# churchill-lab/alntools

Hardware: AMD Instinct MI355X
Metric: alignments/sec BAM->EC (100M PE reads, 8-hap) at 1/2/4/8 MI355X (higher is better)
Workload: dtype u32

## Files before the change

### alntools_amd/csrc/ecb.hip

```cpp
#include <hip/hip_runtime.h>

#include <algorithm>
#include <climits>
#include <cstddef>
#include <cstdarg>
#include <cstdio>
#include <cstring>
#include <cstdlib>
#include <memory>
#include <mutex>
#include <string>
#include <vector>

#include "../../include/ecb.h"

namespace {

typedef unsigned long long u64;
typedef unsigned int u32;
typedef unsigned short u16;

constexpr int TPB = 256;
constexpr u32 MAX_PROBE = 256;
constexpr u32 PENDING = 0xFFFFFFFFu;
constexpr u32 ARENA_CHUNK = 512;
constexpr u32 QSTRIPES = 64;
constexpr u32 ARENA_REGIONS = 64;
constexpr u32 MAX_LOCI = (1u << 26) - 2u;
constexpr u32 MAX_LOCI_SHORT = (1u << 25) - 2u;
constexpr u32 INL = 5;
constexpr u32 DEAD_KEY = 0xFFFFFFFFu;
constexpr u32 SPIN_MAX = 1u << 16;

constexpr u32 ERR_CONTRACT = 1u;
constexpr u32 ERR_RANGE = 2u;
constexpr u32 ERR_ARENA = 4u;
constexpr u32 ERR_QUEUE = 8u;
constexpr u32 ERR_INTERNAL = 16u;
constexpr u32 ERR_COUNT = 32u;

struct alignas(64) Slot {
    u64 lo;
    u32 n1;
    u32 off;
    u32 count;
    u32 first_inv;
    uint2 pair[INL];
};
static_assert(sizeof(Slot) == 64, "one EC per 64-byte line");
static_assert(offsetof(Slot, n1) == 8 && offsetof(Slot, off) == 12 && offsetof(Slot, count) == 16 && offsetof(Slot, first_inv) == 20,
              "k_count_bins reads {n1, off} and {count, first_inv} as 8-byte words");
struct Entry {
    u64 lo, reserved;
    u32 count, first_inv;
    u32 off, n;
};
static_assert(sizeof(Entry) == 32, "exchange format");

struct Counters {
    u64 all, valid;
    u64 arena_top;
    u64 n_queue;
    u64 n_queue_s[QSTRIPES];
    u64 n_ecs;
    u32 err;
    u32 full;
    u64 arena_reg[ARENA_REGIONS];
    u64 next_slice;
    u64 n_mismatch;
    u32 last_rid, pad_;
    u64 n_probe_tiles;
};

__host__ __device__ __forceinline__ u32 arena_regions(u64 arena_cap) { return (u32)(arena_cap >> 16 >= ARENA_REGIONS ? ARENA_REGIONS : (arena_cap >> 16 ? arena_cap >> 16 : 1)); }
__device__ __forceinline__ u64 arena_alloc(Counters* ctr, u64 arena_cap, u32 n, u32 hint) {
    const u32 R = arena_regions(arena_cap);
    const u64 per = arena_cap / R;
    for (u32 t = 0; t < R; ++t) {
        const u32 r = (hint + t) % R;
        const u64 at = atomicAdd(&ctr->arena_reg[r], (u64)n);
        if (at + n <= (u64)(r + 1) * per) return at;
    }
    return ~0ull;
}

__device__ __forceinline__ u32 fmix32(u32 h) {
    h ^= h >> 16; h *= 0x85EBCA6Bu;
    h ^= h >> 13; h *= 0xC2B2AE35u;
    h ^= h >> 16;
    return h;
}
__device__ __forceinline__ u64 pair_hash64(u32 locus, u32 mask) {
    const u32 h0 = fmix32(locus * 0x9E3779B1u + mask * 0x85EBCA77u + 0x7F4A7C15u);
    const u32 h1 = fmix32((h0 ^ locus) * 0xC2B2AE3Du + mask);
    return ((u64)h1 << 32) | h0;
}
__device__ __forceinline__ u64 finish_hash(u64 s0, u32 n) { return (s0 + ((u64)n << 32) + n) | 1ull; }

__device__ __forceinline__ bool rec_valid(u32 hf) {
    if (hf & 0x4u) return false;
    if (hf & 0x1u) {
        if ((hf & 0x80u) || !(hf & 0x2u) || (hf & (ECB_FLAG_MATE_OTHER_REF | ECB_FLAG_NEXT_POS_NEG))) return false;
    }
    return true;
}

enum { ST_NONE = 0, ST_LOOK, ST_HIT, ST_CREATED, ST_PENDING, ST_FULL, ST_OTHER, ST_STUCK };
enum { CMP_EQUAL = 0, CMP_DIFFERENT, CMP_INCOMPLETE, CMP_UNSURE };
struct SlotView { u32 n, off; uint2 p[INL]; };

__device__ __forceinline__ u64 fresh64(u64* p) { return atomicOr(p, 0ull); }
__device__ __forceinline__ void store_wt64(u64* p, u64 v) { __hip_atomic_store(p, v, __ATOMIC_RELAXED, __HIP_MEMORY_SCOPE_AGENT); }
__device__ __forceinline__ u64 pack2(uint2 v) { return ((u64)v.y << 32) | v.x; }
__device__ __forceinline__ uint2 unpack2(u64 v) { return make_uint2((u32)v, (u32)(v >> 32)); }
__device__ __forceinline__ void publish_key(Slot* s, u32 n1, u32 off) { store_wt64(reinterpret_cast<u64*>(&s->n1), ((u64)off << 32) | n1); }
__device__ __forceinline__ uint2 key_pair(const Slot& s, const uint2* arena, u32 i) { return i < INL ? s.pair[i] : arena[(u64)s.off + (i - INL)]; }
__device__ __forceinline__ uint2 key_pair_fresh(Slot* s, uint2* arena, u32 off, u32 i) {
    return unpack2(fresh64(reinterpret_cast<u64*>(i < INL ? &s->pair[i] : arena + ((u64)off + (i - INL)))));
}

__device__ __forceinline__ SlotView make_view(uint4 a, uint4 b, uint4 c, uint4 d) {
    SlotView v;
    v.n = a.z - 1u; v.off = a.w;
    v.p[0] = make_uint2(b.z, b.w); v.p[1] = make_uint2(c.x, c.y); v.p[2] = make_uint2(c.z, c.w);
    v.p[3] = make_uint2(d.x, d.y); v.p[4] = make_uint2(d.z, d.w);
    return v;
}
constexpr u32 RANKED_MAX = 16;
template <class F>
__device__ __forceinline__ void ranked_pairs(const SlotView& v, const uint2* arena, F&& emit) {
    const u32 sn = v.n;
    u32 X[RANKED_MAX], Y[RANKED_MAX];
#pragma unroll
    for (u32 i = 0; i < INL; ++i) { X[i] = i < sn ? v.p[i].x : 0xFFFFFFFFu; Y[i] = v.p[i].y; }
    if (sn <= INL) {
#pragma unroll
        for (u32 i = 0; i < INL; ++i) {
            u32 r = 0;
#pragma unroll
            for (u32 j = 0; j < INL; ++j) r += X[j] < X[i] ? 1u : 0u;
            if (i < sn) emit(r, X[i], Y[i]);
        }
    } else {
#pragma unroll
        for (u32 k = 0; k < RANKED_MAX - INL; ++k) {
            const uint2 t = INL + k < sn ? arena[(u64)v.off + k] : make_uint2(0xFFFFFFFFu, 0u);
            X[INL + k] = t.x; Y[INL + k] = t.y;
        }
#pragma unroll
        for (u32 i = 0; i < RANKED_MAX; ++i) {
            u32 r = 0;
#pragma unroll
            for (u32 j = 0; j < RANKED_MAX; ++j) r += X[j] < X[i] ? 1u : 0u;
            if (i < sn) emit(r, X[i], Y[i]);
        }
    }
}
constexpr u32 BIG_LDS = 2048;
template <class F>
__device__ __forceinline__ void ranked_pairs_wave(const Slot& s, const uint2* arena, u32 sn, u32* sx, u32 lane, F&& emit) {
    const bool in_lds = sn <= BIG_LDS;
    if (in_lds) {
        for (u32 i = lane; i < sn; i += 64) sx[i] = key_pair(s, arena, i).x;
        __builtin_amdgcn_fence(__ATOMIC_ACQ_REL, "wavefront");
        __builtin_amdgcn_wave_barrier();
    }
    for (u32 i = lane; i < sn; i += 64) {
        const uint2 pi = key_pair(s, arena, i);
        u32 r = 0;
        if (in_lds) {
            u32 j = 0;
            for (; j + 4u <= sn; j += 4u) {
                const uint4 v = *reinterpret_cast<const uint4*>(&sx[j]);
                r += (v.x < pi.x ? 1u : 0u) + (v.y < pi.x ? 1u : 0u) + (v.z < pi.x ? 1u : 0u) + (v.w < pi.x ? 1u : 0u);
            }
            for (; j < sn; ++j) r += sx[j] < pi.x ? 1u : 0u;
        } else {
            for (u32 j = 0; j < sn; ++j) r += key_pair(s, arena, j).x < pi.x;
        }
        emit(r, pi.x, pi.y);
    }
    if (in_lds) {
        __builtin_amdgcn_fence(__ATOMIC_ACQ_REL, "wavefront");
        __builtin_amdgcn_wave_barrier();
    }
}
template <class Cmp>
__device__ __forceinline__ int table_lookup(Slot* table, u64 cap_mask, u64 lo, u64& j, u32& probes, const Cmp& cmp, u32 abl = 0u, u32* first_inv_seen = nullptr) {
    for (; probes < MAX_PROBE; ++probes, j = (j + 1) & cap_mask) {
        Slot* s = table + j;
// ... 2253 lines not shown
    HIPCHK(h, hipMemsetAsync(&h->ctr->full, 0, sizeof(u32), h->stream));
    HIPCHK(h, hipMemsetAsync(&h->ctr->next_slice, 0, sizeof(u64), h->stream));
    return ECB_OK;
}

int launch_stream(ecb_handle* h, StreamVariant v, const StreamPlan& P, const u32* d_rid, const u32* d_loc, const u32* d_hf, const int* d_pos, u64 n,
                  u32 prev_rid, const u32* d_last, u32 launch, u64 offered, u64* timing = nullptr) {
    const bool verify = v == SV_VERIFY;
    int2* const rng = verify ? nullptr : (int2*)h->rng;
    u64* d_resume = nullptr; u32* d_wcounts = nullptr;
    POOL(h, P_RESUME, d_resume, 2 * P.slices);
    if (!launch) k_init_resume<<<nblk(P.slices, TPB), TPB, 0, h->stream>>>(d_resume, P.slices, P.chunk, verify ? nullptr : (Counters*)h->ctr);
    POOL(h, P_WCOUNTS, d_wcounts, 3 * P.pwaves);
    if (launch) RCCHK(zero_launch_words(h));
    else {
        if (verify) {
            HIPCHK(h, hipMemsetAsync(d_wcounts, 0, 3 * P.pwaves * sizeof(u32), h->stream));
            RCCHK(zero_launch_words(h));
            HIPCHK(h, hipMemsetAsync(&h->ctr->n_mismatch, 0, sizeof(u64), h->stream));
        } else if (h->wave_arena_n < P.pwaves) {
            HIPCHK(h, h->wave_arena.grow(2 * P.pwaves * sizeof(u64), 0, 2 * h->wave_arena_n * sizeof(u64), h->stream));
            h->wave_arena_n = P.pwaves;
        }
        *h->pin_cold = StreamCold{h->arena, h->arena_cap, h->queue, h->queue_cap, d_resume, d_wcounts, verify ? nullptr : (u64*)h->wave_arena, timing,
                                  P.chunk, prev_rid, d_pos, rng, verify ? 0u : h->cfg.n_loci, verify ? 0u : h->cfg.n_haplotypes};
        HIPCHK(h, hipMemcpyAsync(h->d_cold, h->pin_cold.get(), sizeof(StreamCold), hipMemcpyHostToDevice, h->stream));
    }
    const StreamArgs a{d_rid, d_loc, d_hf, n, h->table, h->cap - 1, h->ctr, h->read_slot, h->run.reads_hi, h->d_cold,
                       !verify && getenv("ECB_ABLATE") ? (u32)atoi(getenv("ECB_ABLATE")) : 0u, d_pos, rng};
    if (h->prof && !verify) hipEventRecord(h->ev0, h->stream);
    STREAM_VARIANTS[v].kernel<<<(unsigned)P.blocks, TPB, 0, h->stream>>>(a);
    if (h->prof && !verify) hipEventRecord(h->ev1, h->stream);
    k_sum_counts<<<1, 1024, 0, h->stream>>>(d_wcounts, P.pwaves, h->ctr, verify ? 1u : 0u, offered, h->queue_cap, d_last);
    HIPCHK(h, hipGetLastError());
    if (!verify) h->last_variant = v;
    return ECB_OK;
}

int verify_pass(ecb_handle* h, const StreamPlan& P, const u32* d_rid, const u32* d_loc, const u32* d_hf, u64 n, u32 prev_rid, u64* n_long, u32 tw) {
    RCCHK(launch_stream(h, SV_VERIFY, P, d_rid, d_loc, d_hf, nullptr, n, prev_rid, nullptr, 0, 0));
    RCCHK(sync_counters(h));
    return run_deferred(h, d_rid, d_loc, d_hf, n, true, tw, n_long);
}
int verify_batch(ecb_handle* h, const u32* d_rid, const u32* d_loc, const u32* d_hf, u64 n, u32 prev_rid, u64* n_mismatch, u64* n_long, u32 tw = 512u) {
    StreamPlan P;
    RCCHK(plan_stream(h, n, &P, SV_VERIFY));
    u64 nq = 0;
    if (const int rc = verify_pass(h, P, d_rid, d_loc, d_hf, n, prev_rid, &nq, tw); rc != ECB_OK) {
        if (h->hctr.err) {
            const std::string refusal = h->err;
            HIPCHK(h, hipMemsetAsync(&h->ctr->err, 0, sizeof(u32), h->stream));
            HIPCHK(h, hipMemsetAsync(&h->ctr->n_queue, 0, (1 + QSTRIPES) * sizeof(u64), h->stream));
            h->hctr.err = 0; h->hctr.n_queue = 0;
            h->err = refusal;
        }
        return rc;
    }
    *n_mismatch = h->hctr.n_mismatch;
    *n_long = nq;
    HIPCHK(h, hipMemsetAsync(&h->ctr->n_queue, 0, (1 + QSTRIPES) * sizeof(u64), h->stream));
    h->hctr.n_queue = 0;
    return ECB_OK;
}

int build_batch(ecb_handle* h, const u32* d_rid, const u32* d_loc, const u32* d_hf, const int* d_pos, u64 n, u32 tw, bool* launched) {
    if (n == 0) return ECB_OK;
    const bool hinted = h->reads_hint != 0;
    u32 last_rid = 0;
    u64 reads_after = std::max<u64>(h->reads_hint, h->run.n_reads);
    if (!hinted) {
        HIPCHK(h, hipMemcpyAsync(&last_rid, d_rid + rec_at(n - 1, tw), sizeof(u32), hipMemcpyDeviceToHost, h->stream));
        HIPCHK(h, hipStreamSynchronize(h->stream));
        reads_after = (u64)(u32)(last_rid + 1u);
        if (reads_after < h->run.n_reads) return fail(h, ECB_ERR_CONTRACT, "read_id went backwards across pushes");
    }
    RCCHK(ensure_read_slot(h, reads_after));
    h->run.reads_hi = reads_after;
    while (h->n_ecs() * 2 > h->cap) { RCCHK(grow_table(h, h->cap * 4)); }
    const StreamVariant v = pick_variant(h, n);
    StreamPlan P;
    RCCHK(plan_stream(h, n, &P, v));
    u64* timing = nullptr;
#ifdef ECB_TIMING
    HIPCHK(h, hipMalloc(&timing, 8 * sizeof(u64)));
    HIPCHK(h, hipMemset(timing, 0, 8 * sizeof(u64)));
#endif
    h->ctr_synced = false;
    *launched = true;
    const u64 probe_before = h->hctr.n_probe_tiles;
    int rc = ECB_OK;
    for (u32 launch = 0;; ++launch) {
        rc = launch_stream(h, v, P, d_rid, d_loc, d_hf, d_pos, n, h->run.prev_rid, d_rid + rec_at(n - 1, tw), launch, launch ? 0 : n, timing);
        if (rc != ECB_OK) break;
        rc = sync_counters(h);
        if (h->prof) {
            float ms = 0; hipEventElapsedTime(&ms, h->ev0, h->ev1);
            h->prof_ms += ms; h->prof_launches += 1;
        }
        if (rc != ECB_OK) break;
        const bool parked = h->hctr.full != 0;
        rc = run_deferred(h, d_rid, d_loc, d_hf, n, false, tw);
        if (rc != ECB_OK) break;
        if (!parked) break;
        rc = grow_table(h, h->cap * 4);
        if (rc != ECB_OK) break;
    }
#ifdef ECB_TIMING
    {
        u64 t[8];
        hipMemcpy(t, timing, sizeof(t), hipMemcpyDeviceToHost); hipFree(timing);
        static const char* nm[8] = {"(a) filter+heads", "tile decisions", "prefetch issue+clear+geometry", "(b) LDS tables", "hash entries", "(c) lookup", "publish/settle/slot stores", "-"};
        u64 tot = 0; for (int i = 0; i < 7; ++i) tot += t[i];
        fprintf(stderr, "[ecb timing] %llu waves, clocks per wave:", (unsigned long long)P.slices);
        for (int i = 0; i < 7; ++i) fprintf(stderr, "  %s %.0f (%.1f%%)", nm[i], (double)t[i] / P.slices, 100.0 * t[i] / std::max<u64>(tot, 1));
        fprintf(stderr, "  tile visits on the probe-on path %llu of %llu tiles", (unsigned long long)t[7], (unsigned long long)((n + WT - 1) / WT));
        fprintf(stderr, "\n");
    }
#endif
    RCCHK(rc);
    {
        const u64 tiles = (n + WT - 1) / WT, on_path = h->hctr.n_probe_tiles - probe_before;
        if (on_path * 4 > tiles) h->par_stream = true; else if (on_path * 16 < tiles) h->par_stream = false;
    }
    if (h->prof) h->prof_records += n;
    if (h->cfg.flags & ECB_F_VERIFY) {
        u64 bad = 0, nl = 0;
        RCCHK(verify_batch(h, d_rid, d_loc, d_hf, n, h->run.prev_rid, &bad, &nl, tw));
        h->run.n_mismatch += bad;
        if (bad) return fail(h, ECB_ERR_VERIFY, "exactness pass: %llu read(s) of this batch sit in an EC whose key is not their target set", (unsigned long long)bad);
    }
    if (hinted) {
        last_rid = h->hctr.last_rid;
        reads_after = (u64)(u32)(last_rid + 1u);
        if (reads_after < h->run.n_reads) return fail(h, ECB_ERR_CONTRACT, "read_id went backwards across pushes");
    }
    h->run.prev_rid = last_rid;
    h->run.n_reads = reads_after;
    h->run.records_pushed += n;
    return ECB_OK;
}
int process_batch(ecb_handle* h, const u32* d_rid, const u32* d_loc, const u32* d_hf, const int* d_pos, u64 n, u32 tw = 512u) {
    bool launched = false;
    const int rc = build_batch(h, d_rid, d_loc, d_hf, d_pos, n, tw, &launched);
    return launched ? run_refused(h, rc) : rc;
}

int ensure_staging(ecb_handle* h, u64 need) {
    if (need <= h->st_cap) return ECB_OK;
    h->st_loc = h->st_hf = nullptr; h->st_pos = nullptr; h->st_cap = 0;
    const u64 cap = std::max<u64>(need, h->cfg.max_batch_records);
    const u64 stride = (cap * sizeof(u32) + (2ull << 20) - 1) / (2ull << 20) * (2ull << 20) / sizeof(u32);
    const bool rg = (h->cfg.flags & ECB_F_RANGES) != 0;
    HIPCHK(h, h->st_rid.alloc((rg ? 4 : 3) * stride * sizeof(u32)));
    h->st_cap = cap;
    h->st_loc = h->st_rid + stride; h->st_hf = h->st_rid + 2 * stride;
    if (rg) h->st_pos = reinterpret_cast<int*>(h->st_rid + 3 * stride);
    return ECB_OK;
}

int stage_and_process(ecb_handle* h, const u32* rid, const u32* loc, const u32* hf, const int* pos, u64 m) {
    const u64 nc = h->run.c_rid.size();
    const u64 n = nc + m;
    if (!n) return ECB_OK;
    RCCHK(ensure_staging(h, n));
    const bool rg = (h->cfg.flags & ECB_F_RANGES) != 0;
    const struct { void* st; const void *carry, *window; } streams[4] = {
        {h->st_rid, h->run.c_rid.data(), rid}, {h->st_loc, h->run.c_loc.data(), loc}, {h->st_hf, h->run.c_hf.data(), hf}, {h->st_pos, h->run.c_pos.data(), pos}};
    for (int w = 0; w < 2; ++w)
        for (int i = 0; i < (rg ? 4 : 3) && (w ? m : nc); ++i)
            HIPCHK(h, hipMemcpyAsync((u32*)streams[i].st + (w ? nc : 0), w ? streams[i].window : streams[i].carry, (w ? m : nc) * 4, hipMemcpyHostToDevice, h->stream));
    HIPCHK(h, hipStreamSynchronize(h->stream));
    h->run.c_rid.clear(); h->run.c_loc.clear(); h->run.c_hf.clear(); h->run.c_pos.clear();
    return process_batch(h, h->st_rid, h->st_loc, h->st_hf, rg ? h->st_pos : nullptr, n);
}

int excl_scan_dev(ecb_handle* h, const u32* in, u64 n, u32* out, u64* d_total, u32 stride = 1, u32* last32 = nullptr) {
    u32* sums = nullptr;
    POOL(h, P_SUMS, sums, scan_words(n));
    HIPCHK(h, scan_launch(h->stream, in, n, out, sums, d_total, stride, last32));
    return ECB_OK;
}
int excl_scan(ecb_handle* h, const u32* in, u64 n, u32* out, u64* total) {
    u64* d_tot = nullptr;
    POOL(h, P_TOTALS, d_tot, 8);
    RCCHK(excl_scan_dev(h, in, n, out, d_tot + 7));
    HIPCHK(h, hipMemcpyAsync(total, d_tot + 7, sizeof(u64), hipMemcpyDeviceToHost, h->stream));
    HIPCHK(h, hipStreamSynchronize(h->stream));
    return ECB_OK;
}

struct SortBufs {
    u64* k[2];
    u32* v[2];
    int at = 0;
    u64* keys() const { return k[at]; }
    u32* vals() const { return v[at]; }
    u64* spare_keys() const { return k[at ^ 1]; }
    u32* spare_vals() const { return v[at ^ 1]; }
// ... 3135 lines not shown
```

### alntools_amd/csrc/k_stream.inc

```
constexpr bool KS_SHORT = ECB_KS_SHORT != 0;
#ifndef ECB_KS_PAR
#define ECB_KS_PAR 0
#endif
constexpr bool KS_PAR = ECB_KS_PAR != 0;
static_assert(!(KS_PAR && KS_SHORT), "one or the other");
constexpr u32 KBITS = KS_SHORT ? 25 : 26;
constexpr u32 KMASK = (1u << KBITS) - 1u;
constexpr int WMAXR = KS_SHORT ? 128 : 64;
#ifndef ECB_WAVES_PER_SIMD
#define ECB_WAVES_PER_SIMD 5
#endif
#ifndef ECB_LGMAX
#define ECB_LGMAX 6
#endif
#ifndef ECB_EST_MUL
#define ECB_EST_MUL 4
#endif
constexpr int WAVES_PER_SIMD = KS_SHORT ? 4 : ECB_WAVES_PER_SIMD;
constexpr int LGMAX = KS_SHORT ? 7 : ECB_LGMAX;
static_assert(LGMAX >= 0 && (1 << LGMAX) <= WMAXR && KBITS + LGMAX <= 32, "a read's index within the pass: the bits of an LDS key above KBITS");
constexpr int CMAX = KS_SHORT ? 64 : 80;
#ifndef ECB_TSLOTS
#define ECB_TSLOTS (ECB_WAVES_PER_SIMD > 4 ? 640 : 896)
#endif
// ... 130 lines not shown
#pragma unroll
        for (u32 i = 0; i < INL; ++i) {
            const u32 want = tag | (v.p[i].x + 1u);
            const u32 valid = i < v.n ? 1u : 0u, same = t[i].x == want ? 1u : 0u, none = t[i].x == 0u ? 1u : 0u;
            inc |= valid & (v.p[i].y == 0u ? 1u : 0u);
            diff |= valid & (none | (same & (t[i].y != v.p[i].y ? 1u : 0u)));
            moved |= (valid & (same ^ 1u) & (none ^ 1u)) << i;
        }
        }
        if (inc) return CMP_INCOMPLETE;
        if (diff) return CMP_DIFFERENT;
        if (moved) {
#pragma unroll
            for (u32 i = 0; i < INL; ++i) {
                const u32 q2 = probe_slot(tag | (v.p[i].x + 1u), 0u);
                t[i] = tab_get(*L, (moved >> i & 1u) ? q2 : home);
            }
            u32 far = 0;
#pragma unroll
            for (u32 i = 0; i < INL; ++i) {
                const u32 want = tag | (v.p[i].x + 1u);
                const u32 m = moved >> i & 1u, same = t[i].x == want ? 1u : 0u, none = t[i].x == 0u ? 1u : 0u;
                diff |= m & (none | (same & (t[i].y != v.p[i].y ? 1u : 0u)));
                far |= (m & (same ^ 1u) & (none ^ 1u)) << i;
            }
            if (diff) return CMP_DIFFERENT;
            while (far) {
                const u32 i = (u32)__builtin_ctz(far);
                far &= far - 1u;
                uint2 pr = v.p[0];
#pragma unroll
                for (u32 k = 1; k < INL; ++k) if (i == k) pr = v.p[k];
                if (!has(pr)) return CMP_DIFFERENT;
            }
        }
        for (u32 i0 = INL; i0 < v.n; i0 += 4u) {
            u64 w[4];
#pragma unroll
            for (u32 k = 0; k < 4u; ++k)
                w[k] = __hip_atomic_load(reinterpret_cast<u64*>(cold->arena + (u64)v.off + (min(i0 + k, v.n - 1u) - INL)), __ATOMIC_RELAXED, __HIP_MEMORY_SCOPE_AGENT);
            for (u32 k = 0; k < 4u && i0 + k < v.n; ++k) {
                const uint2 pr = unpack2(k == 0u ? w[0] : k == 1u ? w[1] : k == 2u ? w[2] : w[3]);
                if (pr.y == 0u) return CMP_INCOMPLETE;
                if (pr.x >= KMASK || !has(pr)) return CMP_DIFFERENT;
            }
        }
        return CMP_EQUAL;
    }
    __device__ __forceinline__ int full(Slot* s, u32 n, u32 off) const {
        if (n != np) return CMP_DIFFERENT;
        for (u32 i = 0; i < n; ++i) {
            uint2 pr = i < INL ? s->pair[i] : cold->arena[(u64)off + (i - INL)];
            if (pr.y == 0u) pr = key_pair_fresh(s, cold->arena, off, i);
            if (pr.y == 0u) return CMP_INCOMPLETE;
            if (pr.x >= KMASK) return CMP_DIFFERENT;
            const u32 key = tag | (pr.x + 1u);
            u32 q = home + home_off(pr.x + 1u, H);
            bool found = false;
            for (u32 it = 0; it < (u32)TSLOTS; ++it) {
                const uint2 t = tab_get(*L, q);
                if (t.x == key) { found = t.y == pr.y; break; }
                if (t.x == 0u) break;
                q = next_slot(key, q, it);
            }
            if (!found) return CMP_DIFFERENT;
        }
        return CMP_EQUAL;
    }
};

template <bool VERIFY, bool RANGES = false>
__global__ __launch_bounds__(TPB, RANGES ? (WAVES_PER_SIMD < 4 ? WAVES_PER_SIMD : 4) : WAVES_PER_SIMD) void k_stream(StreamArgs A) {
    __shared__ WaveLds wl[NWAVE];
    const u32 lane = threadIdx.x & 63u, w = threadIdx.x >> 6;
    WaveLds& L = wl[w];
    const u64 pw = (u64)blockIdx.x * NWAVE + w;
    const StreamCold* const C = A.cold;
    static_assert(WT == 512, "tile index = record index >> 9");
    u32 my_valid = 0, my_new = 0;
    u32 bad = 0;
    if (lane == 0) L.ws[7] = 0u;
    if (!VERIFY && lane == 0) { const u64* wa = C->wave_arena; const u64 ca = wa[2 * pw]; L.ws[2] = (u32)ca; L.ws[3] = (u32)(ca >> 32); L.ws[4] = (u32)wa[2 * pw + 1]; }
#ifdef ECB_TIMING
    u64 tacc[8] = {0, 0, 0, 0, 0, 0, 0, 0}, tlast = __builtin_readcyclecounter();
#endif
    auto clear_pass = [&](u32 ln) {
        uint4* z = tab_base(L);
        u32 zz;
        asm volatile("v_mov_b32 %0, 0" : "=v"(zz));
        const uint4 zv = make_uint4(zz, zz, zz, zz);
#pragma unroll
        for (int t = 0; t < TAB_BYTES / (16 * 64); ++t) z[t * 64 + ln] = zv;
        if constexpr (KS_SHORT) { reinterpret_cast<uint4*>(L.acc)[ln] = zv; reinterpret_cast<u32*>(L.npair)[ln] = zz; }
        else { *reinterpret_cast<uint2*>(&L.acc[ln]) = make_uint2(zz, zz); L.npair[ln] = (unsigned short)zz; }
    };
    clear_pass(lane);
    wave_sync();
  for (;;) {
    u32 wid = 0;
    if (lane == 0) wid = (u32)atomicAdd(&A.ctr->next_slice, 1ull);
    wid = (u32)__builtin_amdgcn_readfirstlane((int)wid);
    const u64 chunk = C->chunk;
    const u64 c0 = (u64)wid * chunk;
    if (c0 >= A.n) break;
    const u64 c1 = min(c0 + chunk, A.n);
    const u64 p = C->resume[2 * (u64)wid], counted0 = C->resume[2 * (u64)wid + 1];
    if (p >= A.n || p == ~0ull) continue;
    u32 tix = (u32)(p >> 9);
    const u32 c1t = (u32)((c1 + (u64)(WT - 1)) >> 9);
    const u32 last_t = (u32)((A.n - 1) >> 9);
    const u32 last_rel = (u32)(A.n - ((u64)last_t << 9));
    const u32 counted_t = (u32)((counted0 + (u64)(WT - 1)) >> 9);
    int p_rel = (int)(p - ((u64)tix << 9));
    u32 prev = p == 0 ? C->prev_rid : A.rid[rec_at(p - 1, A_TW(A))];
    u32 pb = prev + 1u, npend = 0, n_ent = 0;
    ws_put64(L, 5, p, lane);
    bool open = false;
    u32 carry_n = 0;
    u32 lgf = pack_lgf(LGMAX);
    bool revisit = false;
    TileRegs R;
    load_tile(A, (u64)tix << 9, min(((u64)tix << 9) + (u64)WT, A.n), lane, R);
    int r_pos[RANGES ? RPL : 1];
    if constexpr (RANGES) load_pos(A.pos, (u64)tix << 9, min(((u64)tix << 9) + (u64)WT, A.n), lane, r_pos);
    u32 parked = __hip_atomic_load(&A.ctr->full, __ATOMIC_RELAXED, __HIP_MEMORY_SCOPE_AGENT);
    asm volatile("" : "+v"(parked));
    bool slice_done = false;

    while (!slice_done) {
        if (__builtin_amdgcn_readfirstlane((int)parked)) break;
        u32 ln = lane;
        asm volatile("" : "+v"(ln));
        tix = (u32)__builtin_amdgcn_readfirstlane((int)tix);
        prev = (u32)__builtin_amdgcn_readfirstlane((int)prev);
        pb = (u32)__builtin_amdgcn_readfirstlane((int)pb);
        npend = (u32)__builtin_amdgcn_readfirstlane((int)npend);
        n_ent = (u32)__builtin_amdgcn_readfirstlane((int)n_ent);
        lgf = (u32)__builtin_amdgcn_readfirstlane((int)lgf);
        const u32 lg = lgf >> 24;
        const u32 gp = ((u32)TBASE >> lg) + (TSLOTS == 896 ? (256u >> lg) : 0u) + ((u32)(TBASE / 4) >> lg);
        const HomeGeo HG = home_geo(lgf);
        bool do_flush = false, again = false, more = false;
        bool preflush = false;
        bool taken = false;
        u32 parked_next = parked;
        u32 last_pos = 0xFFFFFFFFu;
        u32 last_rid = prev;
        u32 est = 64;
        const bool ends = tix == last_t;
        const bool own = tix < c1t;
        const int te_rel = ends ? (int)last_rel : WT;
        const bool count_tile = own && tix >= counted_t && !revisit;
        const bool plain = p_rel == 0 && te_rel == WT;
        u32 r_key[RPL], r_bit[RPL];
        u32 m_act = 0, m_head = 0;
        const u32 lim = own ? (1u << lg) : (open ? npend + 1u : 0u);
        const u32 rid_first = (u32)__builtin_amdgcn_readfirstlane((int)R.rr[0]), rid_last = (u32)__builtin_amdgcn_readlane((int)R.rr[RPL - 1], 63);
        const bool all_mine = rid_first - pb < lim && rid_last - pb < lim && rid_last >= rid_first;
        {
#pragma unroll
            for (int g = 0; g < NG; ++g) {
                const int i0 = g * 256 + 4 * (int)ln;
                const u32 up = lane_above(R.rr[4 * g + 3]);
                const u32 wrap = g == 0 ? prev : (u32)__builtin_amdgcn_readlane((int)R.rr[4 * (g > 0 ? g - 1 : 0) + 3], 63);
                u32 in4 = 0xFu, te4 = 0xFu;
                if (!plain) {
                    te4 = (1u << clamp04(te_rel - i0, 0, 4)) - 1u;
// ... 144 lines not shown
                for (;;) {
                    if (!from_home) {
                        if (!__ballot(cb != 0u)) break;
                        wave_sync();
                        u32 n_st = 0;
#pragma unroll
                        for (int k = 0; k <= RPL; ++k) {
                            const bool c = cb >> k & 1u;
                            const u64 mm = __ballot(c);
                            if (!mm) continue;
                            const u32 at = n_st + __builtin_amdgcn_mbcnt_hi((u32)(mm >> 32), __builtin_amdgcn_mbcnt_lo((u32)mm, 0u));
                            if (c && at < (u32)CMAX) {
                                const u32 key = k < RPL ? r_key[k < RPL ? k : 0] : c_key, bit = k < RPL ? r_bit[k < RPL ? k : 0] : c_bit;
                                L.carry[at] = make_uint2(key, bit);
                                cb &= ~(1u << k);
                            }
                            n_st = min(n_st + (u32)__popcll(mm), (u32)CMAX);
                        }
                        lo_ = 0u; hi_ = n_st;
                        wave_sync();
                    }
                    for (u32 base = lo_; base < hi_; base += 64u) {
                        const bool have = base + ln < hi_;
                        const uint2 rec = L.carry[have ? base + ln : 0u];
                        bool todo = have, made = false;
                        u32 it = from_home ? 0xFFFFFFFFu : 0u, qq = 0;
                        while (__ballot(todo)) {
                            if (todo) {
                                qq = it == 0xFFFFFFFFu ? (rec.x >> KBITS) * gp + home_off(rec.x, HG) : probe_slot(rec.x, it);
                                const u32 o = atomicCAS(tab_key(L, qq), 0u, rec.x);
                                if (o == 0u || o == rec.x) { todo = false; made = o == 0u; tab_or(L, qq, rec.y); }
                                else if (++it == (u32)TSLOTS) { bad |= ERR_INTERNAL; todo = false; }
                            }
                        }
                        const u64 mm = __ballot(made);
                        if (made) L.ent[n_ent + __builtin_amdgcn_mbcnt_hi((u32)(mm >> 32), __builtin_amdgcn_mbcnt_lo((u32)mm, 0u))] =
                            (unsigned short)(KS_SHORT ? qq : (qq | ((rec.x >> KBITS) << SBITS)));
                        n_ent += (u32)__popcll(mm);
                    }
                    from_home = false;
                }
            }
            carry_n = 0;
        }
        TICK(3);
        do_flush = (npend != 0u || open) &&
                   (!more || again || n_ent + n_mine > (u32)(WT + CMAX) || npend + (open ? 1u : 0u) + n_new > (1u << lg));
        }

        bool giant = false;
        u32 new_carry = 0;
        if (do_flush) {
            wave_sync();
            u32 cn = 0;
            const u32 rl_last = npend;
            const bool keep = open;
            for (u32 e0 = 0; e0 < n_ent; e0 += 64) {
                const u32 e = e0 + ln;
                const bool have = e < n_ent;
                const u32 en = have ? L.ent[e] : 0u, qq = en & SMASK;
                const uint2 en2 = tab_get(L, qq);
                const u32 rl = KS_SHORT ? en2.x >> KBITS : en >> SBITS;
                const bool kept = have && keep && rl == rl_last;
                if (have && !kept) {
                    atomicAdd(&L.acc[rl], pair_hash64((en2.x & KMASK) - 1u, en2.y));
                    atomicAdd(reinterpret_cast<u32*>(&L.npair[rl & ~1u]), (rl & 1u) ? 0x10000u : 1u);
                }
                if (keep) {
                    const u64 mm = __ballot(kept);
                    const u32 at = cn + __builtin_amdgcn_mbcnt_hi((u32)(mm >> 32), __builtin_amdgcn_mbcnt_lo((u32)mm, 0u));
                    if (kept && at < (u32)CMAX) L.carry[at] = make_uint2(en2.x & KMASK, en2.y);
                    cn += (u32)__popcll(mm);
                }
            }
            if (keep) { new_carry = cn; giant = cn > (u32)CMAX; }
            wave_sync();

            TICK(4);
            const u32 nhalf = KS_SHORT ? ((u32)__builtin_amdgcn_readfirstlane((int)npend) + 63u) >> 6 : 1u;
          for (u32 half = 0; half < nhalf; ++half) {
            u64 j = 0;
            u32 st = ST_NONE, probes = 0, np = 0, fseen = 0;
            u64 lo = 0;
            const u32 rx = KS_SHORT ? ln + (half << 6) : ln;
            const bool on = rx < npend && !ABL(A, 3u);
            const u32 rd = pb + rx;
            LdsSetCmp cmp;
            cmp.L = &L; cmp.cold = C; cmp.home = rx * gp; cmp.H = HG; cmp.tag = rx << KBITS; cmp.np = 0;
            if (on) {
                np = L.npair[rx];
                cmp.np = np;
                lo = finish_hash(L.acc[rx], np);
                j = lo & A.cap_mask;
                if ((u64)rd >= A.reads_hi) bad |= ERR_CONTRACT;
                else st = ST_LOOK;
            }
            if (VERIFY) {
                if (st == ST_LOOK) {
                    const u32 sl = A.read_slot[rd];
                    bool same = false;
                    if (sl != PENDING) {
                        const uint4* q = reinterpret_cast<const uint4*>(A.table + sl);
                        const uint4 a = q[0], b = q[1], c = q[2], d = q[3];
                        if (a.z != 0u && a.z != DEAD_KEY) {
                            int r = cmp.quick(make_view(a, b, c, d));
                            if (r == CMP_UNSURE) r = cmp.full(A.table + sl, a.z - 1u, a.w);
                            same = r == CMP_EQUAL;
                        }
                    }
                    if (!same) my_new += 1;
                }
                parked = parked_next; taken = true;
                        } else {
                for (u32 round = 0;; ++round) {
                    if (st == ST_LOOK) {
                        if (ABL(A, 64u)) { st = ST_HIT; fseen = 0xFFFFFFFFu; }
                        else if (ABL(A, 4u)) st = ST_HIT;
                        else st = table_lookup(A.table, A.cap_mask, lo, j, probes, cmp, ABL(A, 24u), &fseen);
                    }
                    if (round == 0u && half == 0u) {
                        TICK(5);
                        parked = parked_next; taken = true;
                    #pragma unroll
                        for (int k = 0; k < RPL; ++k) {
                            asm volatile("" : "+v"(R.rr[k])); asm volatile("" : "+v"(R.ll[k])); asm volatile("" : "+v"(R.hh[k]));
                            if constexpr (RANGES) asm volatile("" : "+v"(r_pos[k]));
                        }
                        asm volatile("" : "+v"(parked));
                    }
                    const u64 cmask = __ballot(st == ST_CREATED);
                    if (cmask) {
                        const bool cr = st == ST_CREATED;
                        const u32 want = cr && np > INL ? np - INL : 0u;
                        u32 off = 0;
                        if (__ballot(want != 0u)) {
                            const u32 incl = wave_incl_scan(want);
                            const u32 total = (u32)__builtin_amdgcn_readlane((int)incl, 63);
                            u64 chunk_at = ws_get64(L, 2);
                            u32 chunk_left = (u32)__builtin_amdgcn_readfirstlane((int)L.ws[4]);
                            if (total > chunk_left) {
                                const u32 take = max(total, ARENA_CHUNK);
                                u64 at = 0;
                                if (ln == 0) at = arena_alloc(A.ctr, C->arena_cap, take, (u32)pw);
                                chunk_at = ((u64)(u32)__builtin_amdgcn_readfirstlane((int)(u32)(at >> 32)) << 32) | (u32)__builtin_amdgcn_readfirstlane((int)(u32)at);
                                chunk_left = take;
                                if (chunk_at == ~0ull) { bad |= ERR_ARENA; chunk_left = 0; }
                            }
                            if (!(bad & ERR_ARENA)) {
                                off = (u32)(chunk_at + (incl - want));
                                chunk_at += total; chunk_left -= total;
                            }
                            ws_put64(L, 2, chunk_at, ln);
                            if (ln == 0) L.ws[4] = chunk_left;
                        }
                        const bool dead = (bad & ERR_ARENA) != 0u;
                        const u32 j32 = (u32)j;
                        uint2* const arena = C->arena;
                        if (!dead) for (u32 e0 = 0; e0 < n_ent; e0 += 64) {
                            const u32 e = e0 + ln;
                            const u32 en = e < n_ent ? L.ent[e] : 0u, qq = en & SMASK;
                            const u32 rl = KS_SHORT ? tab_get(L, qq).x >> KBITS : en >> SBITS;
                            const u32 o = __shfl(off, rl & 63u), jj = __shfl(j32, rl & 63u);
                            if (e < n_ent && (!KS_SHORT || (rl >> 6) == half) && (cmask >> (rl & 63u) & 1ull) && !ABL(A, 32u)) {
                                const u32 was = atomicSub(reinterpret_cast<u32*>(&L.npair[rl & ~1u]), (rl & 1u) ? 0x10000u : 1u);
                                const u32 pos = ((rl & 1u) ? was >> 16 : was & 0xFFFFu) - 1u;
                                uint2* dst = pos < INL ? &A.table[jj].pair[pos] : arena + ((u64)o + (pos - INL));
                                const uint2 en2 = tab_get(L, qq);
                                store_wt64(reinterpret_cast<u64*>(dst), pack2(make_uint2((en2.x & KMASK) - 1u, en2.y)));
                            }
                        }
                        if (cr) { publish_key(A.table + j, dead ? DEAD_KEY : np + 1u, off); st = ST_HIT; }
                        my_new += (u32)__popcll(cmask);
                    }
                    if (!__ballot(st == ST_PENDING)) break;
                    if (round >= 64u) { if (st == ST_PENDING) { bad |= ERR_INTERNAL; st = ST_NONE; } break; }
                    if (st == ST_PENDING) {
                        const int r = table_settle(A.table + j, cmp);
                        if (r == ST_HIT) st = ST_HIT;
                        else if (r == ST_STUCK) { bad |= ERR_INTERNAL; st = ST_NONE; atomicExch(&A.ctr->full, 1u); }
                        else { j = (j + 1) & A.cap_mask; ++probes; st = ST_LOOK; }
                    }
                }
                if (st == ST_FULL) {
                    atomicExch(&A.ctr->full, 1u);
                    queue_defer(A.ctr, C, tile_head(A.rid, (u64)wid * C->chunk, min(((u64)tix << 9) + (u64)WT, A.n), rd, A_TW(A)));
                } else if (st == ST_HIT) {
                    A.read_slot[rd] = (u32)j;
                    if (~rd > fseen) atomicMax(&A.table[j].first_inv, ~rd);
                }
            }
          }
            wave_sync();
            clear_pass(ln);
            pb += npend; npend = 0; n_ent = 0;
            const u32 e4 = min(est * (u32)ECB_EST_MUL, 1u << LGMAX);
            lgf = pack_lgf(e4 > 1u ? 32u - (u32)__builtin_clz(e4 - 1u) : 0u);
            if (open) {
                if (!giant) carry_n = new_carry;
                else {
                    if (ln == 0) {
                        queue_defer(A.ctr, C, ws_get64(L, 0));
                    }
                    open = false; pb += 1u;
                }
            }
            ws_put64(L, 5, open ? ws_get64(L, 0) : (u64)((preflush || again) ? tix : tix + 1u) << 9, ln);
            wave_sync();
            TICK(6);
        }
        if (preflush) { revisit = true; continue; }
        if (!taken) {
            parked = parked_next;
        #pragma unroll
            for (int k = 0; k < RPL; ++k) {
                asm volatile("" : "+v"(R.rr[k])); asm volatile("" : "+v"(R.ll[k])); asm volatile("" : "+v"(R.hh[k]));
                if constexpr (RANGES) asm volatile("" : "+v"(r_pos[k]));
            }
            asm volatile("" : "+v"(parked));
        }
        if (again) { revisit = true; continue; }
        revisit = false; p_rel = 0;
        prev = last_rid;
        slice_done = !more;
        tix += 1u;
    }
    u64 p_out = ws_get64(L, 5);
    const u64 counted = max(counted0, min((u64)(revisit ? tix + 1u : tix) << 9, c1));
    const bool stopped = __ballot(bad != 0u) || __builtin_amdgcn_readfirstlane((int)parked);
    if (__ballot(bad != 0u)) { if (bad) atomicOr(&A.ctr->err, bad); p_out = ~0ull; }
    else if (slice_done) p_out = ~0ull;
    if (lane == 0) { u64* rs = C->resume; rs[2 * (u64)wid] = p_out; rs[2 * (u64)wid + 1] = counted; }
    if (stopped) break;
  }
    const u32 wa = (u32)__builtin_amdgcn_readfirstlane((int)L.ws[7]), wv = wave_sum(my_valid);
    const u32 wn = VERIFY ? wave_sum(my_new) : my_new;
#ifdef ECB_TIMING
    if (lane == 0 && C->timing) for (int i = 0; i < 8; ++i) atomicAdd(C->timing + i, tacc[i]);
#endif
    if (lane == 0) { u32* wc = C->wave_counts; wc[3 * pw] = wa; wc[3 * pw + 1] = wv; wc[3 * pw + 2] = wn; }
    if (!VERIFY && lane == 0) { u64* wav = C->wave_arena; wav[2 * pw] = ((u64)L.ws[3] << 32) | L.ws[2]; wav[2 * pw + 1] = L.ws[4]; }
}
```

Baseline: 334.6 billion.

## Inline hash-table probe as wave-lockstep look/claim loop with overlapped slot loads

Replaces the per-lane table_lookup call with an inline loop in which every lane that is still looking or claiming advances one step per iteration. Each step issues the 64-byte slot load and the claim CAS together, so divergent probe chains run in lockstep across the wave instead of serially inside the helper. The first iteration also carries the existing prefetch-retire barrier block, overlapping it with the lookup. Timing-only counters for table trips and claim-only rounds are added, and the settle path now caps probes at MAX_PROBE, which adds extra ballots and register pressure in exchange.

```diff
diff --git a/alntools_amd/csrc/ecb.hip b/alntools_amd/csrc/ecb.hip
--- a/alntools_amd/csrc/ecb.hip
+++ b/alntools_amd/csrc/ecb.hip
@@ -105,7 +105,7 @@
     return true;
 }
 
-enum { ST_NONE = 0, ST_LOOK, ST_HIT, ST_CREATED, ST_PENDING, ST_FULL, ST_OTHER, ST_STUCK };
+enum { ST_NONE = 0, ST_LOOK, ST_HIT, ST_CREATED, ST_PENDING, ST_FULL, ST_OTHER, ST_STUCK, ST_CLAIM };
 enum { CMP_EQUAL = 0, CMP_DIFFERENT, CMP_INCOMPLETE, CMP_UNSURE };
 struct SlotView { u32 n, off; uint2 p[INL]; };
 
@@ -2525,8 +2525,8 @@
     RCCHK(plan_stream(h, n, &P, v));
     u64* timing = nullptr;
 #ifdef ECB_TIMING
-    HIPCHK(h, hipMalloc(&timing, 8 * sizeof(u64)));
-    HIPCHK(h, hipMemset(timing, 0, 8 * sizeof(u64)));
+    HIPCHK(h, hipMalloc(&timing, 16 * sizeof(u64)));
+    HIPCHK(h, hipMemset(timing, 0, 16 * sizeof(u64)));
 #endif
     h->ctr_synced = false;
     *launched = true;
@@ -2550,13 +2550,16 @@
     }
 #ifdef ECB_TIMING
     {
-        u64 t[8];
+        u64 t[16];
         hipMemcpy(t, timing, sizeof(t), hipMemcpyDeviceToHost); hipFree(timing);
         static const char* nm[8] = {"(a) filter+heads", "tile decisions", "prefetch issue+clear+geometry", "(b) LDS tables", "hash entries", "(c) lookup", "publish/settle/slot stores", "-"};
         u64 tot = 0; for (int i = 0; i < 7; ++i) tot += t[i];
         fprintf(stderr, "[ecb timing] %llu waves, clocks per wave:", (unsigned long long)P.slices);
         for (int i = 0; i < 7; ++i) fprintf(stderr, "  %s %.0f (%.1f%%)", nm[i], (double)t[i] / P.slices, 100.0 * t[i] / std::max<u64>(tot, 1));
         fprintf(stderr, "  tile visits on the probe-on path %llu of %llu tiles", (unsigned long long)t[7], (unsigned long long)((n + WT - 1) / WT));
+        fprintf(stderr, "  table trips per lookup %.3f (claim-only %.3f) over %llu lookups: 1: %.1f%%  2: %.1f%%  3: %.1f%%  4+: %.1f%%", (double)t[12] / std::max<u64>(t[14], 1),
+                (double)t[13] / std::max<u64>(t[14], 1), (unsigned long long)t[14], 100.0 * t[8] / std::max<u64>(t[14], 1), 100.0 * t[9] / std::max<u64>(t[14], 1),
+                100.0 * t[10] / std::max<u64>(t[14], 1), 100.0 * t[11] / std::max<u64>(t[14], 1));
         fprintf(stderr, "\n");
     }
 #endif
diff --git a/alntools_amd/csrc/k_stream.inc b/alntools_amd/csrc/k_stream.inc
--- a/alntools_amd/csrc/k_stream.inc
+++ b/alntools_amd/csrc/k_stream.inc
@@ -236,7 +236,7 @@
     if (lane == 0) L.ws[7] = 0u;
     if (!VERIFY && lane == 0) { const u64* wa = C->wave_arena; const u64 ca = wa[2 * pw]; L.ws[2] = (u32)ca; L.ws[3] = (u32)(ca >> 32); L.ws[4] = (u32)wa[2 * pw + 1]; }
 #ifdef ECB_TIMING
-    u64 tacc[8] = {0, 0, 0, 0, 0, 0, 0, 0}, tlast = __builtin_readcyclecounter();
+    u64 tacc[16] = {0, 0, 0, 0, 0, 0, 0, 0, 0, 0, 0, 0, 0, 0, 0, 0}, tlast = __builtin_readcyclecounter();
 #endif
     auto clear_pass = [&](u32 ln) {
         uint4* z = tab_base(L);
@@ -547,6 +547,9 @@
             u64 j = 0;
             u32 st = ST_NONE, probes = 0, np = 0, fseen = 0;
             u64 lo = 0;
+#ifdef ECB_TIMING
+            u32 f_rounds = 0, f_claim = 0;
+#endif
             const u32 rx = KS_SHORT ? ln + (half << 6) : ln;
             const bool on = rx < npend && !ABL(A, 3u);
             const u32 rd = pb + rx;
@@ -581,17 +584,55 @@
                     if (st == ST_LOOK) {
                         if (ABL(A, 64u)) { st = ST_HIT; fseen = 0xFFFFFFFFu; }
                         else if (ABL(A, 4u)) st = ST_HIT;
-                        else st = table_lookup(A.table, A.cap_mask, lo, j, probes, cmp, ABL(A, 24u), &fseen);
-                    }
-                    if (round == 0u && half == 0u) {
-                        TICK(5);
-                        parked = parked_next; taken = true;
-                    #pragma unroll
-                        for (int k = 0; k < RPL; ++k) {
-                            asm volatile("" : "+v"(R.rr[k])); asm volatile("" : "+v"(R.ll[k])); asm volatile("" : "+v"(R.hh[k]));
-                            if constexpr (RANGES) asm volatile("" : "+v"(r_pos[k]));
-                        }
-                        asm volatile("" : "+v"(parked));
+                    }
+                    for (bool first = round == 0u && half == 0u;; first = false) {
+                        const bool look = st == ST_LOOK, claim = st == ST_CLAIM;
+#ifdef ECB_TIMING
+                        if (__ballot(look || claim)) { f_rounds += 1u; if (!__ballot(look)) f_claim += 1u; }
+#endif
+                        Slot* const s = A.table + j;
+                        const uint4* const q = reinterpret_cast<const uint4*>(look ? s : A.table);
+                        uint4 a = q[0], b = a, c = a, d = a;
+                        if (!ABL(A, 16u)) { b = q[1]; c = q[2]; d = q[3]; }
+                        u64 got = 0;
+                        if (claim) got = atomicCAS(&s->lo, 0ull, lo);
+                        asm volatile("" : "+v"(a.x), "+v"(a.y), "+v"(a.z), "+v"(a.w), "+v"(b.x), "+v"(b.y), "+v"(b.z), "+v"(b.w));
+                        asm volatile("" : "+v"(c.x), "+v"(c.y), "+v"(c.z), "+v"(c.w), "+v"(d.x), "+v"(d.y), "+v"(d.z), "+v"(d.w), "+v"(got));
+                        bool adv = false;
+                        if (look) {
+                            fseen = 0u;
+                            const u64 clo = ((u64)a.y << 32) | a.x;
+                            if (clo == 0ull) st = ST_CLAIM;
+                            else if (clo != lo) adv = true;
+                            else if (a.z == 0u) st = ST_PENDING;
+                            else if (a.z == DEAD_KEY) adv = true;
+                            else {
+                                fseen = b.y;
+                                if (ABL(A, 8u)) st = ST_HIT;
+                                else {
+                                    const int r = cmp.quick(make_view(a, b, c, d));
+                                    if (r == CMP_EQUAL) st = ST_HIT;
+                                    else if (r == CMP_DIFFERENT) adv = true;
+                                    else st = ST_PENDING;
+                                }
+                            }
+                        } else if (claim) {
+                            if (got == 0ull) st = ST_CREATED;
+                            else if (got == lo) st = ST_PENDING;
+                            else adv = true;
+                        }
+                        if (adv) { j = (j + 1) & A.cap_mask; ++probes; st = probes < MAX_PROBE ? ST_LOOK : ST_FULL; }
+                        if (first) {
+                            TICK(5);
+                            parked = parked_next; taken = true;
+                        #pragma unroll
+                            for (int k = 0; k < RPL; ++k) {
+                                asm volatile("" : "+v"(R.rr[k])); asm volatile("" : "+v"(R.ll[k])); asm volatile("" : "+v"(R.hh[k]));
+                                if constexpr (RANGES) asm volatile("" : "+v"(r_pos[k]));
+                            }
+                            asm volatile("" : "+v"(parked));
+                        }
+                        if (!__ballot(st == ST_LOOK || st == ST_CLAIM)) break;
                     }
                     const u64 cmask = __ballot(st == ST_CREATED);
                     if (cmask) {
@@ -639,13 +680,19 @@
                     }
                     if (!__ballot(st == ST_PENDING)) break;
                     if (round >= 64u) { if (st == ST_PENDING) { bad |= ERR_INTERNAL; st = ST_NONE; } break; }
+#ifdef ECB_TIMING
+                    f_rounds += 1u;
+#endif
                     if (st == ST_PENDING) {
                         const int r = table_settle(A.table + j, cmp);
                         if (r == ST_HIT) st = ST_HIT;
                         else if (r == ST_STUCK) { bad |= ERR_INTERNAL; st = ST_NONE; atomicExch(&A.ctr->full, 1u); }
-                        else { j = (j + 1) & A.cap_mask; ++probes; st = ST_LOOK; }
-                    }
-                }
+                        else { j = (j + 1) & A.cap_mask; ++probes; st = probes < MAX_PROBE ? ST_LOOK : ST_FULL; }
+                    }
+                }
+#ifdef ECB_TIMING
+                tacc[8] += f_rounds <= 1u; tacc[9] += f_rounds == 2u; tacc[10] += f_rounds == 3u; tacc[11] += f_rounds >= 4u; tacc[12] += f_rounds; tacc[13] += f_claim; tacc[14] += 1;
+#endif
                 if (st == ST_FULL) {
                     atomicExch(&A.ctr->full, 1u);
                     queue_defer(A.ctr, C, tile_head(A.rid, (u64)wid * C->chunk, min(((u64)tix << 9) + (u64)WT, A.n), rd, A_TW(A)));
@@ -700,7 +747,7 @@
     const u32 wa = (u32)__builtin_amdgcn_readfirstlane((int)L.ws[7]), wv = wave_sum(my_valid);
     const u32 wn = VERIFY ? wave_sum(my_new) : my_new;
 #ifdef ECB_TIMING
-    if (lane == 0 && C->timing) for (int i = 0; i < 8; ++i) atomicAdd(C->timing + i, tacc[i]);
+    if (lane == 0 && C->timing) for (int i = 0; i < 16; ++i) atomicAdd(C->timing + i, tacc[i]);
 #endif
     if (lane == 0) { u32* wc = C->wave_counts; wc[3 * pw] = wa; wc[3 * pw + 1] = wv; wc[3 * pw + 2] = wn; }
     if (!VERIFY && lane == 0) { u64* wav = C->wave_arena; wav[2 * pw] = ((u64)L.ws[3] << 32) | L.ws[2]; wav[2 * pw + 1] = L.ws[4]; }
```

New measurement: 355.1 billion (median of 6 runs). +6.1%, better.
